# alibasaran/die-e

Hardware: AMD Instinct MI355X
Metric: self-play games/sec (higher is better)
Workload: dtype bf16

## Files before the change

die-e_amd/csrc/mcts_kernels.hip:

```cpp
#include <hip/hip_runtime.h>
#include <stdint.h>

#include <algorithm>
#include <type_traits>

#include "bg_device.h"
#include "nn_device.h"
#include "launch.h"
#include "mcts_device.h"
#include "search_iter_device.h"
#include "search_types.h"
#include "wave_ops.h"

namespace diee {

__device__ __forceinline__ void backprop(const Tree& T, size_t base, uint32_t idx, float v) {
    while (idx != kNone) {
        T.visits[base + idx] += 1.0f;
        T.value[base + idx] += v;
        idx = T.parent[base + idx];
    }
}

__device__ __forceinline__ void backprop_path(const Tree& T, size_t base, uint32_t my_node, int lane, uint32_t len, float v) {
// ... 419 lines not shown
            cn[SC_EXPANSIONS] += 1; cn[SC_CHILDREN] += (uint32_t)k;
            if ((uint32_t)k > cn[SC_MAX_CHILDREN]) cn[SC_MAX_CHILDREN] = (uint32_t)k;
        }
    }
    }
    EX_STAMP(4);
    meet();
    EX_STAMP(5);
    if constexpr (!TWO) bp_section();
    }
    };
    if constexpr (!TWO) commit();
    if constexpr (TWO == 2) {
        if (!main_wave) {
            commit();
            if (lane == 0) { sc_all.hand[0] = expanded ? 1u : 0u; sc_all.hand[1] = new_meta; sc_all.hand[2] = new_first; }
            __syncthreads();
            return;
        }
    }
    EX_STAMP(6);
    if (next_it != kNoNext) {
        meet();
        EX_STAMP(7);
        if constexpr (TWO) {
            select_slot(T, S, G, slot, seg, lane, next_it, c, P.quirks, cn, &rh, &l0, [&](uint32_t nd, uint32_t& nm, uint32_t& nf) {
                if (committed || nd != node) return false;
                commit();
                if (!expanded) return false;
                meet();
                nm = new_meta; nf = new_first;
                return true;
            });
        } else {
            select_slot(T, S, G, slot, seg, lane, next_it, c, P.quirks, cn, &rh, &l0);
        }
        EX_STAMP(8);
    }
    if constexpr (TWO) if (!committed) commit();
    if (lane == 0) store_counters(S, slot, cn);
#ifdef DIEE_EXPAND_STAMPS
    if (threadIdx.x == 0) atomicAdd(&g_expand_stamps[15], 1ull);
#endif
}

template <bool PRE, int TWO = 0>
__global__ __launch_bounds__(TWO ? 128 : 64) void k_expand(Tree T, Slots S, Segs G, uint32_t n, uint32_t it, SearchParams P,
                                                           uint32_t next_it, float c) {
    __shared__ ExpandScratchOf<PRE, TWO> sc_all;
    expand_body<PRE, TWO>(T, S, G, n, it, P, next_it, c, blockIdx.x, sc_all);
}

constexpr int kTailSpin = 1 << 20;
__device__ __forceinline__ bool tail_meet(uint32_t* word, uint32_t n, bool hit, int lane, uint32_t* err, uint32_t& misses, bool absent = false) {
    if (n == 1) { misses = hit ? 0u : 1u; return true; }
    __threadfence();
    uint32_t v = 0;
    if (lane == 0) {
        if (!absent) atomicAdd(word, hit ? 1u : 0x10001u);
        int spins = 0;
        for (;;) {
            v = __hip_atomic_load(word, __ATOMIC_RELAXED, __HIP_MEMORY_SCOPE_AGENT);
            if ((v & 0xffffu) >= n) break;
            if (++spins > kTailSpin) { atomicOr(err, 4u); v = 0xffffffffu; break; }
            __builtin_amdgcn_s_sleep(2);
        }
    }
    v = (uint32_t)__builtin_amdgcn_readfirstlane((int)v);
    __builtin_amdgcn_fence(__ATOMIC_ACQUIRE, "agent");
    misses = v >> 16;
    return v != 0xffffffffu;
}

#ifdef DIEE_TAIL_STAMPS
__device__ unsigned long long g_tail_stamps[8];
#define TL_STAMP(i) do { const unsigned long long tn_ = __builtin_readcyclecounter(); if (threadIdx.x == 0) atomicAdd(&g_tail_stamps[i], tn_ - tl_prev_); tl_prev_ = __builtin_readcyclecounter(); } while (0)
#define TL_COUNT(i) do { if (threadIdx.x == 0) atomicAdd(&g_tail_stamps[i], 1ull); } while (0)
extern "C" int diee_dev_tail_stamps(unsigned long long* out, int reset) {
    if (out && hipMemcpyFromSymbol(out, HIP_SYMBOL(g_tail_stamps), sizeof(unsigned long long) * 8) != hipSuccess) return 1;
    if (reset) { unsigned long long z[8] = {0}; if (hipMemcpyToSymbol(HIP_SYMBOL(g_tail_stamps), z, sizeof(z)) != hipSuccess) return 1; }
    return 0;
}
#else
#define TL_STAMP(i) do {} while (0)
#define TL_COUNT(i) do {} while (0)
#endif
struct TailArgs { Tail L; uint32_t q; };

struct TailTree {
    float vis[kTailLdsNodes], val[kTailLdsNodes], pri[kTailLdsNodes], cval[kTailLdsNodes];
    uint32_t meta[kTailLdsNodes], fc[kTailLdsNodes], crow[kTailLdsNodes];
};
struct TailLds {
    TailTree t;
    float vvis[kTailLdsNodes], vval[kTailLdsNodes];
    WaveScratch ws;
    float lgs[22 * 64];
    float raw[kMaxPlays];
    uint16_t code[kMaxPlays];
    uint32_t cand[64];
};
static_assert(sizeof(TailLds) <= 160 * 1024, "one workgroup per CU");

struct TreeLds : StagedStats {
    TailTree& t;
    struct Hdr { uint32_t meta, first_child; __device__ __forceinline__ uint32_t bits() const { return meta; } };
    __device__ __forceinline__ Hdr hdr(uint32_t i) const { return i < cap ? Hdr{t.meta[i], t.fc[i]} : Hdr{T.meta[base + i], T.first_child[base + i]}; }
    __device__ __forceinline__ static uint32_t nch(const Hdr& h) { return meta_nch(h.meta); }
    __device__ __forceinline__ static uint32_t fc(const Hdr& h) { return h.first_child; }
    __device__ __forceinline__ uint32_t leaf_meta(uint32_t, const Hdr& h) const { return h.meta; }
    __device__ __forceinline__ void set_header(uint32_t i, uint32_t m, uint32_t f) const {
        if (i < cap) { t.meta[i] = m; t.fc[i] = f; }
        T.meta[base + i] = m; T.first_child[base + i] = f;
    }
};

__global__ __launch_bounds__(64) void k_tail(Tree T, Slots S, Segs G, uint32_t n, SearchParams P, float c, TailArgs A) {
    extern __shared__ __attribute__((aligned(16))) char tail_smem[];
    uint32_t slot = blockIdx.x;
    if (gridDim.x == 8u * n) { if ((blockIdx.x & 7u) != 0u) return; slot = blockIdx.x >> 3; }
    if (slot >= n) return;
    const Tail& L = A.L;
    const int lane = threadIdx.x;
    if (L.state[1] != 0u) return;
#ifdef DIEE_TAIL_STAMPS
    unsigned long long tl_prev_ = __builtin_readcyclecounter();
#endif
    TL_COUNT(7);
    uint32_t it = L.state[0];
    TailLds& D = *reinterpret_cast<TailLds*>(tail_smem);
    const size_t base = (size_t)slot * T.node_cap;
    uint32_t* crow_g = L.crow + (size_t)slot * T.node_cap;
    float* cval_g = L.cval + (size_t)slot * T.node_cap;
    const TreeLds X{{T, base, kTailLdsNodes, D.t.vis, D.t.val, D.t.pri}, D.t};
    const bool quirks = P.quirks != 0;
    SlotRecord R;
    R.load(T, S, G, slot, lane);
    bool all_sel = false;
    if (quirks && slot == R.seg_first) {
        const uint32_t g = R.seg_first + (uint32_t)lane;
        all_sel = __ballot(g < R.seg_end && S.sel[g] == kNone) == 0ull && R.seg_end - R.seg_first <= 64u;
    }
    const uint32_t nl = R.used < kTailLdsNodes ? R.used : kTailLdsNodes;
    for (uint32_t i = lane; i < nl; i += 64) {
        D.t.vis[i] = T.visits[base + i]; D.t.val[i] = T.value[base + i]; D.t.pri[i] = T.prior[base + i];
        D.t.meta[i] = T.meta[base + i]; D.t.fc[i] = T.first_child[base + i];
        D.t.crow[i] = crow_g[i]; D.t.cval[i] = cval_g[i];
    }
    __syncthreads();
    uint32_t ahead_hi = R.used;
    if (A.q > 0) {
        if (L.child_rows > 0) {
            for (uint32_t i = R.used + (uint32_t)lane; i < R.used + (uint32_t)kMaxPlays && i < kTailLdsNodes; i += 64) { D.t.crow[i] = 0; D.t.cval[i] = 0.0f; }
            __syncthreads();
        }
        const uint32_t pq = A.q - 1, nr = L.n_rows[pq] < L.rows ? L.n_rows[pq] : L.rows;
        for (uint32_t r = lane; r < nr; r += 64) {
            const uint32_t rn = L.rows_node[pq * L.rows + r];
            if ((rn >> 24) == slot) {
                const uint32_t node = rn & 0xFFFFFFu;
                const float cv = row_value(L.hv + (size_t)(pq * L.rows + r) * 72, S.wv);
                cval_g[node] = cv; crow_g[node] = pq * L.rows + r + 1u;
                if (node < kTailLdsNodes) { D.t.cval[node] = cv; D.t.crow[node] = pq * L.rows + r + 1u; }
                if (node >= ahead_hi) ahead_hi = node + 1u;
            }
        }
        ahead_hi = (uint32_t)wave_allmax_i32((int)ahead_hi);
        __syncthreads();
    }
    TL_STAMP(0);
    R.lst = load_state(&S.eval_states[slot]);
    const IterScratch scratch{&D.ws, D.lgs, D.raw, D.code};
    bool hit = false;
    uint32_t misses = 0;
    for (;;) {
        const uint32_t cr = R.lterm ? 0u : (R.leaf < kTailLdsNodes ? D.t.crow[R.leaf] : crow_g[R.leaf]);
        hit = R.lterm || cr != 0u;
        const uint32_t ring = (R.lterm || cr == 0u) ? 0u : cr - 1u;
        NetRowLoaded pre;
        pre.vh = value_head_load(L.hv + (size_t)ring * 72, S.wv, lane);
        softmax_load(L.logits + (size_t)ring * 1352, lane, pre.lg);
        if (!tail_meet(L.bar + it + A.q, n, hit, lane, S.overflow, misses, L.test_skip != 0u && slot == n - 1u && it + A.q + 1u == L.test_skip)) {
            if (lane == 0) { atomicMax(&L.state[1], 2u); L.host[1] = 2u; __threadfence_system(); }
            return;
        }
        TL_STAMP(1);
        if (misses != 0u) break;
        uint2 ifl = make_uint2(1u, 0u);
        if (R.lterm || (quirks && slot == R.seg_first && !all_sel)) ifl = *(const uint2*)(S.iter_flags + 2 * ((size_t)R.seg * G.iter_cap + it));
        search_iteration(S, R, X, pre, scratch, ifl, it, slot, lane, quirks, [&](uint32_t cl, float prj, uint32_t cm) {
            if (cl < kTailLdsNodes) {
                D.t.vis[cl] = 0.0f; D.t.val[cl] = 0.0f; D.t.pri[cl] = prj; D.t.meta[cl] = cm; D.t.fc[cl] = 0;
                if (cl >= ahead_hi) { D.t.crow[cl] = 0; D.t.cval[cl] = 0.0f; }
            }
        });
        if (it + 1 < L.iterations) {
            uint32_t* nflag = S.iter_flags + 2 * ((size_t)R.seg * G.iter_cap + it + 1);
            uint32_t node = 0, depth = 0, mine = lane == 0 ? 0u : kNone;
            TreeLds::Hdr h = X.hdr(0);
            float nvis = X.vis(0);
            for (;;) {
                const uint32_t k = X.nch(h);
                if (k == 0) break;
                node = X.fc(h) + select_level(X, X.fc(h), k, sqrtf(nvis), c, lane);
                ++depth;
                if ((uint32_t)lane == depth) mine = node;
                h = X.hdr(node); nvis = X.vis(node);
            }
            if (end_selection(S, R, X, node, depth, mine, h, lane)) {
                if (lane == 0 && quirks && R.sel == kNone) atomicAdd(&nflag[1], 1u);
            } else {
                R.sel = node;
                if (lane == 0) nflag[0] = 1u;
            }
        }
        ++it;
        __syncthreads();
        TL_STAMP(2); TL_COUNT(6);
        if (it >= L.iterations) break;
    }
    R.store(T, S, slot, lane);
    const bool done = it >= L.iterations;
    uint32_t mine_rows = 0, ncand = 0;
    if (!done) {
        const uint32_t room = L.rows - (misses < L.rows ? misses : L.rows);
        const uint32_t want0 = room / n + (slot < room % n ? 1u : 0u), want = want0 < 63u ? want0 : 63u;
        const uint32_t nu = R.used < kTailLdsNodes ? R.used : kTailLdsNodes;
        const bool redistribute = L.extra_rows > 0 && L.rollout_steps > 0 && n > 1 && room > 0 && room / n < 8u;
        const bool second_round = redistribute || L.child_rows > 0;
        const uint32_t want_x = !redistribute ? want : want + L.extra_rows < 63u ? want + L.extra_rows : 63u;
        if (want_x > 0 && L.rollout_steps > 0) {
            for (uint32_t i = lane; i < nu; i += 64) { D.vvis[i] = D.t.vis[i]; D.vval[i] = D.t.val[i]; }
            __syncthreads();
            const uint32_t demanded = hit ? kNone : R.leaf;
            uint32_t fruitless = 0;
            for (uint32_t step = 0; step < L.rollout_steps && ncand < want_x && fruitless < 8; ++step) {
                const VirtualDescent d = virtual_descent<true>(X, D.vvis, D.vval, nu, c, lane);
                const uint32_t node = d.node, cr = node < kTailLdsNodes ? D.t.crow[node] : crow_g[node];
                float x = 0.0f;
                bool fresh = false;
                if (d.bits & kMetaTerminal) x = finished_value(d.bits, R.root_player);
                else if (cr != 0) x = node < kTailLdsNodes ? D.t.cval[node] : cval_g[node];
                else if (!(d.bits & kDrained) && node != demanded) fresh = __ballot((uint32_t)lane < ncand && D.cand[lane] == node) == 0ull;
                if (fresh) { if (lane == 0) D.cand[ncand] = node; ++ncand; fruitless = 0; } else ++fruitless;
                virtual_visit(d, D.vvis, D.vval, nu, x, lane);
                __syncthreads();
            }
        }
        uint32_t nchild = 0;
        if (L.child_rows > 0 && !hit && !(R.leaf_meta & kDrained)) {
            int k = bg_legal_plays_wave(R.lst, &D.ws, lane, S.overflow);
            if (k > kMaxPlays || R.used + (uint32_t)k > T.node_cap) k = 0;
            nchild = (uint32_t)k < L.child_rows ? (uint32_t)k : L.child_rows;
            __syncthreads();
        }
        const uint32_t share = ncand < want ? ncand : want, dem = hit ? 0u : 1u;
        mine_rows = dem + share;
        uint32_t start = 0;
        if (lane == 0 && mine_rows) start = atomicAdd(&L.n_rows[A.q], mine_rows);
        start = (uint32_t)__builtin_amdgcn_readfirstlane((int)start);
        if ((uint32_t)lane < mine_rows && start + (uint32_t)lane < L.rows) {
            const uint32_t node = (dem && lane == 0) ? R.leaf : D.cand[(uint32_t)lane - dem];
            const uint32_t r = A.q * L.rows + start + (uint32_t)lane;
            store_state(&L.rows_state[r], (dem && lane == 0) ? R.lst : load_state(&T.state[base + node]));
            L.rows_node[r] = (slot << 24) | node;
        }
        uint32_t extra = 0;
        if (second_round) {
            uint32_t unused_;
            const bool met = tail_meet(L.bar2 + A.q, n, true, lane, S.overflow, unused_);
            const uint32_t more = redistribute ? ncand - share : 0u;
            extra = met ? nchild + more : 0u;
            uint32_t start2 = 0;
            if (lane == 0 && extra) {
                start2 = atomicAdd(&L.n_rows[A.q], extra);
                const uint32_t fit = start2 >= L.rows ? 0u : extra < L.rows - start2 ? extra : L.rows - start2;
                if (fit < extra) atomicSub(&L.n_rows[A.q], extra - fit);
            }
            start2 = (uint32_t)__builtin_amdgcn_readfirstlane((int)start2);
            extra = start2 >= L.rows ? 0u : extra < L.rows - start2 ? extra : L.rows - start2;
            for (uint32_t j = (uint32_t)lane; j < extra; j += 64) {
                const uint32_t r = A.q * L.rows + start2 + j;
                if (j < nchild) {
                    BgState cs = R.lst;
                    int d0, d1;
                    draw_dice(R.seed, R.gid, R.rnd, it + 1u, j, d0, d1);
                    bg_apply_dev(cs, D.ws.play[j], d0, d1);
                    store_state(&L.rows_state[r], cs);
                    L.rows_node[r] = (slot << 24) | (R.used + j);
                } else {
                    const uint32_t node = D.cand[share + (j - nchild)];
                    store_state(&L.rows_state[r], load_state(&T.state[base + node]));
                    L.rows_node[r] = (slot << 24) | node;
                }
            }
        }
        R.cn[SC_NN_ROWS] += mine_rows + extra;
        if (lane == 0 && share + extra) atomicAdd(&L.state[3], share + extra);
    }
    if (lane == 0) store_counters(S, slot, R.cn);
    TL_STAMP(3);
    if (slot == 0 && lane == 0 && !done) L.n_dem[A.q] = misses;
    if (slot == 0 && lane == 0) {
        const uint32_t was = atomicMax(&L.state[1], done ? 1u : 0u);
        const uint32_t now = was > (done ? 1u : 0u) ? was : (done ? 1u : 0u);
        L.state[0] = it;
        if (!done) L.state[2] += 1u;
        L.host[0] = it; L.host[1] = now; L.host[2] = A.q;
        __threadfence_system();
    }
}

constexpr int kFreeSpinFew = 48, kFreeFewGames = 64;
constexpr uint32_t kFreeRowBits = 12;
struct FreeArgs { Free F; uint32_t q; };
#ifdef DIEE_TAIL_STAMPS
__device__ unsigned long long g_free_stamps[16];
#define FR_STAMP(i) do { const unsigned long long tn_ = __builtin_readcyclecounter(); if (threadIdx.x == 0) atomicAdd(&g_free_stamps[i], tn_ - fr_prev_); fr_prev_ = __builtin_readcyclecounter(); } while (0)
#define FR_COUNT(i, k) do { if (threadIdx.x == 0) atomicAdd(&g_free_stamps[i], (unsigned long long)(k)); } while (0)
extern "C" int diee_dev_free_stamps(unsigned long long* out, int reset) {
    if (out && hipMemcpyFromSymbol(out, HIP_SYMBOL(g_free_stamps), sizeof(unsigned long long) * 16) != hipSuccess) return 1;
    if (reset) { unsigned long long z[16] = {0}; if (hipMemcpyToSymbol(HIP_SYMBOL(g_free_stamps), z, sizeof(z)) != hipSuccess) return 1; }
    return 0;
}
#else
#define FR_STAMP(i) do {} while (0)
#define FR_COUNT(i, k) do {} while (0)
#endif
constexpr uint32_t kFreeLdsNodeBytes = 32;
__host__ __device__ __forceinline__ constexpr uint32_t free_hdr(uint32_t meta, uint32_t first_child) {
    return (meta & 0xE0000000u) | (((meta >> 16) & 0x1ffu) << 20) | (first_child & 0xFFFFFu);
}
__host__ __device__ __forceinline__ constexpr uint32_t hdr_nch(uint32_t h) { return (h >> 20) & 0x1ffu; }
__host__ __device__ __forceinline__ constexpr uint32_t hdr_fc(uint32_t h) { return h & 0xFFFFFu; }
__host__ __device__ constexpr size_t free_lds_bytes(uint32_t ln) {
    return (size_t)ln * kFreeLdsNodeBytes + sizeof(WaveScratch) + sizeof(float) * kMaxPlays + sizeof(uint16_t) * kMaxPlays + sizeof(uint32_t) * 64u;
}
struct TreeF : StagedStats {
    uint32_t* lhdr;
    struct Hdr { uint32_t w; __device__ __forceinline__ uint32_t bits() const { return w; } };
    __device__ __forceinline__ Hdr hdr(uint32_t i) const { return Hdr{i < cap ? lhdr[i] : free_hdr(T.meta[base + i], T.first_child[base + i])}; }
    __device__ __forceinline__ static uint32_t nch(const Hdr& h) { return hdr_nch(h.w); }
    __device__ __forceinline__ static uint32_t fc(const Hdr& h) { return hdr_fc(h.w); }
    __device__ __forceinline__ uint32_t leaf_meta(uint32_t i, const Hdr&) const { return T.meta[base + i]; }
    __device__ __forceinline__ void set_header(uint32_t i, uint32_t m, uint32_t f) const {
        if (i < cap) lhdr[i] = free_hdr(m, f);
        T.meta[base + i] = m; T.first_child[base + i] = f;
    }
};
__device__ __forceinline__ uint32_t free_load(const uint32_t* p) { return __hip_atomic_load(p, __ATOMIC_RELAXED, __HIP_MEMORY_SCOPE_AGENT); }

__global__ __launch_bounds__(64) void k_free(Tree T, Slots S, Segs G, uint32_t n, SearchParams P, float c, FreeArgs A) {
    extern __shared__ __attribute__((aligned(16))) char free_smem[];
    const uint32_t slot = blockIdx.x;
    if (slot >= n) return;
    const Free& F = A.F;
    const int lane = threadIdx.x;
    if (F.state[0] != 0u) return;
    uint32_t it = F.prog[slot];
    if (it >= F.iterations) { if (lane == 0) F.wish_n[slot] = it << 8; return; }
    const uint32_t active0 = A.q == 0 ? n : F.state[4];
    const uint32_t active = active0 ? active0 : 1u;
    const bool few = active * 8u <= n || active <= 8u;
    const uint32_t iter_cap = few ? 64u * F.iter_cap : F.iter_cap;
#ifdef DIEE_TAIL_STAMPS
    unsigned long long fr_prev_ = __builtin_readcyclecounter();
    const unsigned long long fr_t0_ = fr_prev_;
#endif
    FR_COUNT(8, 1);
    const uint32_t ln = F.lds_nodes;
    float* lvis = (float*)free_smem; float* lval = lvis + ln; float* lpri = lval + ln;
    float* vvis = lpri + ln; float* vval = vvis + ln;
    float* lcval = vval + ln;
    uint32_t* lhdr = (uint32_t*)(lcval + ln); uint32_t* lcrow = lhdr + ln;
    WaveScratch& ws = *reinterpret_cast<WaveScratch*>(lcrow + ln);
    float* raw = reinterpret_cast<float*>(&ws + 1);
    uint16_t* code = reinterpret_cast<uint16_t*>(raw + kMaxPlays);
    uint32_t* cand = reinterpret_cast<uint32_t*>(code + kMaxPlays);
    float* lgs = (float*)&ws.keyA[0];
    const size_t base = (size_t)slot * T.node_cap;
    uint32_t* crow_g = F.crow + base;
    float* cval_g = F.cval + base;
    const TreeF X{{T, base, ln, lvis, lval, lpri}, lhdr};
    const bool quirks = P.quirks != 0;
    SlotRecord R;
    R.load(T, S, G, slot, lane);
    uint32_t fsel = 0;
    if (quirks && slot == R.seg_first) {
        uint32_t m = 0;
        for (uint32_t g = R.seg_first + (uint32_t)lane; g < R.seg_end; g += 64) {
            const uint32_t f = F.first_sel[g];
            m = f == kNone ? 0x7fffffffu : (f > m ? f : m);
            if (f == kNone) break;
        }
        fsel = (uint32_t)wave_allmax_i32((int)m);
    }
    const uint32_t nl = R.used < ln ? R.used : ln;
    for (uint32_t i0 = 0; i0 < nl; i0 += 256) {
        float a[4], b[4], p[4], cv4[4]; uint32_t m[4], f[4], r[4];
#pragma unroll
        for (int u = 0; u < 4; ++u) {
            const uint32_t i = i0 + 64u * u + (uint32_t)lane;
            const size_t gi = base + (i < nl ? i : 0u);
// ... 25 lines not shown
    auto batch_progress = [&]() {
        int m = 0x7fffffff;
        for (uint32_t g = R.seg_first + (uint32_t)lane; g < R.seg_end; g += 64) { const int v = (int)free_load(&F.prog[g]); m = v < m ? v : m; }
        return (uint32_t)(-wave_allmax_i32(-m));
    };
    R.lst = load_state(&S.eval_states[slot]);
    const IterScratch scratch{&ws, lgs, raw, code};
    FR_STAMP(0);
    bool have = false, stalled = false;
    uint32_t minprog = 0;
    auto net_row = [&](uint32_t cr_) {
        NetRowLoaded p;
        const size_t ring = (size_t)(((cr_ - 1u) >> kFreeRowBits) % F.ring) * F.rows + ((cr_ - 1u) & ((1u << kFreeRowBits) - 1u));
        p.vh = value_head_load(F.hv + ring * 72, S.wv, lane);
        softmax_load(F.logits + ring * 1352, lane, p.lg);
        return p;
    };
    uint32_t cr = R.lterm ? 0u : crow_of(R.leaf);
    NetRowLoaded pre;
    if (!R.lterm && at_hand(cr)) pre = net_row(cr);
    uint32_t ran = 0;
    for (;; ++ran) {
        have = R.lterm || at_hand(cr);
        if (!have) break;
        if (ran >= iter_cap) { stalled = true; break; }
        uint32_t* iflag = S.iter_flags + 2 * ((size_t)R.seg * G.iter_cap + it);
        const bool need_cnt = quirks && slot == R.seg_first && it < fsel;
        const bool need_any = R.lterm && (quirks || slot == R.seg_first);
        uint2 ifl = make_uint2(1u, 0u);
        if (need_any || need_cnt) {
            bool fin = false;
            const int spins = n <= (uint32_t)kFreeFewGames ? kFreeSpinFew : 1;
            for (int spin = 0; spin < spins; ++spin) {
                if (!need_cnt && (iflag[0] != 0u || free_load(&iflag[0]) != 0u)) { ifl.x = 1u; fin = true; break; }
                if (minprog < it) minprog = batch_progress();
                if (minprog >= it) {
                    ifl.x = free_load(&iflag[0]); ifl.y = free_load(&iflag[1]);
                    fin = true;
                    break;
                }
                __builtin_amdgcn_s_sleep(8);
            }
            if (!fin) { stalled = true; break; }
        }
        FR_STAMP(1);
        search_iteration(S, R, X, pre, scratch, ifl, it, slot, lane, quirks, [&](uint32_t cl, float prj, uint32_t cm) {
            crow_g[cl] = 0u;
            if (cl < ln) { lvis[cl] = 0.0f; lval[cl] = 0.0f; lpri[cl] = prj; lhdr[cl] = free_hdr(cm, 0u); lcrow[cl] = 0; }
        });
        FR_STAMP(2);
        uint32_t published = 0;
        if (it + 1 < F.iterations) {
            uint32_t* nflag = S.iter_flags + 2 * ((size_t)R.seg * G.iter_cap + it + 1);
            uint32_t node = 0, depth = 0, mine = lane == 0 ? 0u : kNone;
            TreeF::Hdr h = X.hdr(0);
            float nvis = X.vis(0);
            for (;;) {
                const uint32_t k = X.nch(h), fcn = X.fc(h);
                if (k == 0) break;
                const float sq = sqrtf(nvis);
                if (k <= 64u && fcn + k <= ln) {
                    const bool valid = (uint32_t)lane < k;
                    const uint32_t ci = fcn + (valid ? (uint32_t)lane : 0u);
                    const float vis = lvis[ci];
                    const uint32_t ch = lhdr[ci];
                    const float sc_ = puct_score(vis, lval[ci], lpri[ci], sq, c);
                    const unsigned long long nans = __ballot(valid && sc_ != sc_);
                    const int lastnan = nans ? 63 - __clzll((long long)nans) : -1;
                    const bool comp = valid && sc_ == sc_ && lane > lastnan;
                    const float mx = wave_allmax_f32(comp ? sc_ : -INFINITY);
                    const unsigned long long win = __ballot(comp && sc_ == mx);
                    const int chosen = win ? 63 - __clzll((long long)win) : lastnan;
                    node = fcn + (uint32_t)chosen;
                    ++depth;
                    if ((uint32_t)lane == depth) mine = node;
                    h.w = (uint32_t)__builtin_amdgcn_readlane((int)ch, chosen);
                    nvis = __builtin_bit_cast(float, __builtin_amdgcn_readlane(__builtin_bit_cast(int, vis), chosen));
                    continue;
                }
                node = fcn + select_level(X, fcn, k, sq, c, lane);
                ++depth;
                if ((uint32_t)lane == depth) mine = node;
                h = X.hdr(node); nvis = X.vis(node);
            }
            if (end_selection(S, R, X, node, depth, mine, h, lane)) {
                if (lane == 0 && quirks && R.sel == kNone) published = atomicAdd(&nflag[1], 1u);
            } else {
                if (lane == 0) {
                    if (nflag[0] == 0u) published = atomicOr(&nflag[0], 1u);
                    if (R.sel == kNone) F.first_sel[slot] = it + 1u;
                }
                R.sel = node;
            }
            cr = R.lterm ? 0u : crow_of(R.leaf);
            if (!R.lterm && at_hand(cr)) pre = net_row(cr);
        }
        ++it;
        __syncthreads();
        if (lane == 0) {
            asm volatile("" :: "v"(published) : "memory");
            atomicExch(&F.prog[slot], it);
        }
        FR_STAMP(3); FR_COUNT(9, 1);
        if (it >= F.iterations) break;
    }
    R.store(T, S, slot, lane);
    const bool done = it >= F.iterations;
    uint32_t nw = 0;
    const bool dem = !done && !stalled && !have;
    if (!done) {
        uint32_t* wl = F.wish + (size_t)slot * kFreeWish;
        if (dem) { if (lane == 0) wl[0] = R.leaf; nw = 1; }
        uint32_t want0 = F.cand_max < kFreeWish - 1u ? F.cand_max : kFreeWish - 1u;
        uint32_t steps_max = F.rollout_steps;
        if (few && want0) {
            const uint32_t room = (F.rows > active ? F.rows - active : 0u) / active;
            want0 = room + 1u < kFreeWish - 1u ? (room + 1u > want0 ? room + 1u : want0) : kFreeWish - 1u;
            steps_max = 2u * F.rollout_steps + 8u;
        }
        const uint32_t want = few ? want0 : (want0 > ran / 2u + 1u ? want0 - ran / 2u : (want0 ? 1u : 0u));
        uint32_t ncand = 0;
        if (want > 0 && steps_max > 0) {
            const uint32_t nu = R.used < ln ? R.used : ln;
            for (uint32_t i0 = 0; i0 < nu; i0 += 256) {
                float a[4], b[4];
#pragma unroll
                for (int u = 0; u < 4; ++u) { const uint32_t i = i0 + 64u * u + (uint32_t)lane; a[u] = lvis[i < nu ? i : 0u]; b[u] = lval[i < nu ? i : 0u]; }
#pragma unroll
                for (int u = 0; u < 4; ++u) { const uint32_t i = i0 + 64u * u + (uint32_t)lane; if (i < nu) { vvis[i] = a[u]; vval[i] = b[u]; } }
            }
            __syncthreads();
            const uint32_t demanded = dem ? R.leaf : kNone;
            uint32_t fruitless = 0;
            const uint32_t h0 = X.hdr(0).w, k0 = hdr_nch(h0), fc0 = hdr_fc(h0);
            const bool resident = R.used <= ln && k0 >= 1u && k0 <= 64u;
            if (resident) {
                auto rl_u = [](uint32_t v_, int l_) { return (uint32_t)__builtin_amdgcn_readlane((int)v_, l_); };
                auto rl_f = [](float v_, int l_) { return __builtin_bit_cast(float, __builtin_amdgcn_readlane(__builtin_bit_cast(int, v_), l_)); };
                const bool rc = (uint32_t)lane < k0;
                const uint32_t rci = fc0 + (rc ? (uint32_t)lane : 0u);
                float r_vis = vvis[0], c_vis = vvis[rci], c_val = vval[rci];
                const float c_pri = lpri[rci], c_cval = lcval[rci];
                const uint32_t c_hdr = lhdr[rci], c_crow = lcrow[rci];
                uint32_t my_cand = kNone;
                for (uint32_t step = 0; step < steps_max && ncand < want && fruitless < 8; ++step) {
                    auto last_max = [&](bool comp, float sc_, uint32_t k_) {
                        const float mx = wave_allmax_f32(comp ? sc_ : -INFINITY);
                        const unsigned long long win = __ballot(comp && sc_ == mx);
                        return win ? 63 - __clzll((long long)win) : (int)k_ - 1;
                    };
                    int j0;
                    {
                        const float sq = __builtin_amdgcn_sqrtf(r_vis);
                        const float sc_ = puct_score_approx(c_vis, c_val, c_pri, sq, c);
                        j0 = last_max(rc && sc_ == sc_, sc_, k0);
                    }
                    uint32_t node = fc0 + (uint32_t)j0, depth = 1, mine = kNone, mt = h0;
                    uint32_t hn = rl_u(c_hdr, j0), ncr = rl_u(c_crow, j0);
                    float pvis = rl_f(c_vis, j0), pval = 0.0f, ncv = rl_f(c_cval, j0), mvis = 0.0f, mval = 0.0f;
                    for (;;) {
                        mt = hn;
                        const uint32_t k = hdr_nch(mt);
                        if (k == 0) break;
                        const uint32_t fcn = hdr_fc(mt);
                        const float sq = __builtin_amdgcn_sqrtf(pvis);
                        if (k <= 64u) {
                            const bool valid = (uint32_t)lane < k;
                            const uint32_t ci = fcn + (valid ? (uint32_t)lane : 0u);
                            const float vis = vvis[ci], val = vval[ci], pr = lpri[ci], cv = lcval[ci];
                            const uint32_t h = lhdr[ci], cr = lcrow[ci];
                            const float sc_ = puct_score_approx(vis, val, pr, sq, c);
                            const int lw = last_max(valid && sc_ == sc_, sc_, k);
                            node = fcn + (uint32_t)lw;
                            hn = rl_u(h, lw); ncr = rl_u(cr, lw); pvis = rl_f(vis, lw); pval = rl_f(val, lw); ncv = rl_f(cv, lw);
                            ++depth;
                            if ((uint32_t)lane == depth) { mine = node; mvis = pvis; mval = pval; }
                            if (depth >= 63) break;
                            continue;
                        }
                        Best b{0.0f, -1};
                        for (uint32_t j = lane; j < k; j += 64) {
                            const uint32_t ci = fcn + j;
                            const float sc_ = puct_score_approx(vvis[ci], vval[ci], lpri[ci], sq, c);
                            if (sc_ == sc_ && (b.j < 0 || !(b.s > sc_))) { b.s = sc_; b.j = (int)j; }
                        }
                        b = wave_best(b);
                        node = fcn + (uint32_t)(b.j >= 0 ? b.j : (int)k - 1);
                        hn = lhdr[node]; ncr = lcrow[node]; pvis = vvis[node]; pval = vval[node]; ncv = lcval[node];
                        ++depth;
                        if ((uint32_t)lane == depth) { mine = node; mvis = pvis; mval = pval; }
                        if (depth >= 63) break;
                    }
                    float x = 0.0f;
                    bool fresh = false;
                    if (mt & kMetaTerminal) x = finished_value(mt, R.root_player);
                    else if (at_hand(ncr)) x = ncv;
                    else if (!(mt & kDrained) && node != demanded) fresh = __ballot((uint32_t)lane < ncand && my_cand == node) == 0ull;
                    if (fresh) { if ((uint32_t)lane == ncand) my_cand = node; if (lane == 0) wl[nw + ncand] = node; ++ncand; fruitless = 0; } else ++fruitless;
                    r_vis += 1.0f;
                    if (lane == j0) { c_vis += 1.0f; c_val += x; }
                    if (lane >= 2 && (uint32_t)lane <= depth) { vvis[mine] = mvis + 1.0f; vval[mine] = mval + x; }
                    __builtin_amdgcn_wave_barrier();
                    FR_COUNT(11, 1);
                }
            } else
            for (uint32_t step = 0; step < steps_max && ncand < want && fruitless < 8; ++step) {
                const VirtualDescent d = virtual_descent<false>(X, vvis, vval, nu, c, lane);
                const uint32_t node = d.node, cr = crow_of(node);
                float x = 0.0f;
                bool fresh = false;
                if (d.bits & kMetaTerminal) x = finished_value(d.bits, R.root_player);
                else if (at_hand(cr)) x = node < ln ? lcval[node] : cval_g[node];
                else if (!(d.bits & kDrained) && node != demanded) fresh = __ballot((uint32_t)lane < ncand && cand[lane] == node) == 0ull;
                if (fresh) { if (lane == 0) { cand[ncand] = node; wl[nw + ncand] = node; } ++ncand; fruitless = 0; } else ++fruitless;
                virtual_visit(d, vvis, vval, nu, x, lane);
                __syncthreads();
                FR_COUNT(11, 1);
            }
        }
        nw += ncand;
    }
    if (lane == 0) {
        F.wish_n[slot] = nw | (it << 8) | (dem ? 0x80000000u : 0u);
        store_counters(S, slot, R.cn);
    }
    FR_STAMP(4);
#ifdef DIEE_TAIL_STAMPS
    if (threadIdx.x == 0) atomicMax(&g_free_stamps[10], __builtin_readcyclecounter() - fr_t0_);
#endif
}

__global__ __launch_bounds__(256) void k_free_first_sel(const uint32_t* __restrict__ sel, uint32_t* __restrict__ first_sel, uint32_t n) {
    const uint32_t g = blockIdx.x * 256u + threadIdx.x;
    if (g < n) first_sel[g] = sel[g] == kNone ? kNone : 0u;
}

__global__ __launch_bounds__(1024) void k_free_pack(Free F, uint32_t n, uint32_t node_cap, uint32_t q, const BgState* __restrict__ arena) {
    const uint32_t kBoost = F.lag_boost < kFreeBoostMax ? F.lag_boost : kFreeBoostMax, kLagStep = F.lag_step ? F.lag_step : 1u;
    __shared__ uint32_t hist[kFreeWish + kFreeBoostMax + 2];
    __shared__ uint32_t wsum[16];
    __shared__ uint32_t s_full, s_rem, s_dem, s_undone, s_maxprog;
    const int tid = threadIdx.x, lane = tid & 63, wave = tid >> 6;
    if (F.state[0] != 0u) return;
    if (tid < (int)(kFreeWish + kFreeBoostMax + 2)) hist[tid] = 0;
    if (tid == 0) { s_dem = 0; s_undone = 0; s_maxprog = 0; }
    __syncthreads();
    const uint32_t rot = (q * 131u) % n;
    const uint32_t g = (uint32_t)tid < n ? ((uint32_t)tid + rot) % n : 0u;
    const uint32_t w = (uint32_t)tid < n ? F.wish_n[g] : ((F.iterations) << 8);
    const uint32_t cnt = (w & 0xffu) < kFreeWish ? (w & 0xffu) : kFreeWish, dem = (w >> 31) < cnt ? (w >> 31) : cnt, spec = cnt - dem, prog = (w >> 8) & 0x7fffffu;
    const bool undone = prog < F.iterations;
    if ((uint32_t)tid < n && undone) { atomicMax(&s_maxprog, prog); atomicAdd(&s_undone, 1u); if (dem) atomicAdd(&s_dem, 1u); }
    __syncthreads();
    const uint32_t lag = undone ? s_maxprog - prog : 0u;
    const uint32_t shift = kBoost - (lag / kLagStep < kBoost ? lag / kLagStep : kBoost);
    if ((uint32_t)tid < n) for (uint32_t r = 1; r <= spec; ++r) atomicAdd(&hist[r + shift], 1u);
    __syncthreads();
// ... 446 lines not shown
```

die-e_amd/csrc/search_iter_device.h:

```cpp
#pragma once
#include <hip/hip_runtime.h>
#include <stdint.h>

#include "bg_device.h"
#include "mcts_device.h"
#include "nn_device.h"
#include "search_types.h"
#include "wave_ops.h"

namespace diee {

__device__ __forceinline__ float puct_score(float vis, float val, float pr, float sq, float c) {
    const float q = vis == 0.0f ? 0.0f : val / vis;
    const float t = sq / (vis + 1.0f);
    const float u = c * t;
    const float w = u * pr;
    return q + w;
}
__device__ __forceinline__ float puct_score_approx(float vis, float val, float pr, float sq, float c) {
    const float q = vis == 0.0f ? 0.0f : val * __builtin_amdgcn_rcpf(vis);
    return q + (c * (sq * __builtin_amdgcn_rcpf(vis + 1.0f))) * pr;
}

struct Best { float s; int j; };
// ... 149 lines not shown
#pragma unroll
        for (int q = 0; q < 22; ++q) sc.lgs[lane + 64 * q] = pre.lg[q];
        __syncthreads();
        for (int j = lane; j < k; j += 64) {
            const uint32_t cd = bg_encode_dev(r0, r1, sc.ws->play[j]);
            sc.raw[j] = softmax_prob(sc.lgs[cd], smM, smInv); sc.code[j] = (uint16_t)cd;
        }
        __syncthreads();
        float pr[4];
#pragma unroll
        for (int r = 0; r < 4; ++r) pr[r] = lane + 64 * r < k ? sc.raw[lane + 64 * r] : 0.0f;
        float sum = 0.0f;
#pragma unroll
        for (int r = 0; r < 4; ++r) {
            const int kr = k - 64 * r < 64 ? k - 64 * r : 64;
            for (int j = 0; j < kr; ++j) sum += __builtin_bit_cast(float, __builtin_amdgcn_readlane(__builtin_bit_cast(int, pr[r]), j));
        }
        const uint32_t first = R.used;
        if (first + (uint32_t)k > T.node_cap) {
            if (lane == 0) atomicOr(S.overflow, 2u);
        } else {
            const uint32_t e = it + 1u;
            for (int j = lane; j < k; j += 64) {
                const uint32_t cl = first + (uint32_t)j;
                const size_t ci = X.base + cl;
                BgState cs = R.lst;
                int d0, d1;
                draw_dice(R.seed, R.gid, R.rnd, e, (uint32_t)j, d0, d1);
                bg_apply_dev(cs, sc.ws->play[j], d0, d1);
                store_state(&T.state[ci], cs);
                const float prj = sc.raw[j] / sum;
                const uint32_t cm = (uint32_t)sc.code[j] | meta_terminal_bits(cs);
                T.visits[ci] = 0.0f; T.value[ci] = 0.0f; T.prior[ci] = prj;
                T.parent[ci] = R.leaf; T.first_child[ci] = 0; T.meta[ci] = cm;
                on_child(cl, prj, cm);
            }
            const uint32_t nmeta = kDrained | ((uint32_t)k << 16) | (m0 & kMetaKeep);
            if (lane == 0) X.set_header(R.leaf, nmeta, first);
            R.used = first + (uint32_t)k;
            R.cn[SC_EXPANSIONS] += 1; R.cn[SC_CHILDREN] += (uint32_t)k;
            if ((uint32_t)k > R.cn[SC_MAX_CHILDREN]) R.cn[SC_MAX_CHILDREN] = (uint32_t)k;
        }
        __syncthreads();
    }
    if (!R.lterm) backprop_selection(X, R.plen, R.pnode, R.leaf, v, lane);
    if (quirks && slot == R.seg_first && ifl.y != 0u && lane == 0) {
        float rvis = X.vis(0), rval = X.val(0);
        for (uint32_t i = 0; i < ifl.y; ++i) { rvis += 1.0f; rval += R.rv0; }
        X.set_stats(0, rvis, rval);
    }
    __syncthreads();
}

template <class TreeX>
__device__ __forceinline__ bool end_selection(const Slots& S, SlotRecord& R, const TreeX& X, uint32_t node, uint32_t depth, uint32_t mine,
                                              const typename TreeX::Hdr& h, int lane) {
    const uint32_t npl = depth < S.path_cap ? depth + 1u : 0u;
    R.cn[SC_SELECTIONS] += 1; R.cn[SC_DEPTH_SUM] += depth;
    if (h.bits() & kMetaTerminal) {
        backprop_selection(X, npl, mine, node, finished_value(h.bits(), R.root_player), lane);
        R.cn[SC_TERMINAL] += 1;
        R.lterm = true;
        return true;
    }
    R.lterm = false; R.leaf = node; R.plen = npl; R.pnode = mine;
    R.leaf_meta = X.leaf_meta(node, h);
    R.lst = load_state(&X.T.state[X.base + node]);
    return false;
}

struct VirtualDescent { uint32_t node, depth, mine, bits; };
template <bool EXACT, class TreeX>
__device__ __forceinline__ VirtualDescent virtual_descent(const TreeX& X, const float* vvis, const float* vval, uint32_t nu, float c, int lane) {
    VirtualDescent d{0u, 0u, lane == 0 ? 0u : kNone, 0u};
    for (;;) {
        const typename TreeX::Hdr h = X.hdr(d.node);
        d.bits = h.bits();
        const uint32_t k = X.nch(h);
        if (k == 0) break;
        const uint32_t fcn = X.fc(h);
        const float nv = d.node < nu ? vvis[d.node] : X.T.visits[X.base + d.node];
        const float sq = EXACT ? sqrtf(nv) : __builtin_amdgcn_sqrtf(nv);
        Best b{0.0f, -1};
        for (uint32_t j = lane; j < k; j += 64) {
            const uint32_t ci = fcn + j;
            const float vis = ci < nu ? vvis[ci] : X.T.visits[X.base + ci], val = ci < nu ? vval[ci] : X.T.value[X.base + ci];
            const float sc_ = EXACT ? puct_score(vis, val, X.pri(ci), sq, c) : puct_score_approx(vis, val, X.pri(ci), sq, c);
            if (sc_ == sc_ && (b.j < 0 || !(b.s > sc_))) { b.s = sc_; b.j = (int)j; }
        }
        b = wave_best(b);
        d.node = fcn + (uint32_t)(b.j >= 0 ? b.j : (int)k - 1);
        ++d.depth;
        if ((uint32_t)lane == d.depth) d.mine = d.node;
        if (d.depth >= 63) break;
    }
    return d;
}
__device__ __forceinline__ void virtual_visit(const VirtualDescent& d, float* vvis, float* vval, uint32_t nu, float x, int lane) {
    if ((uint32_t)lane <= d.depth && d.mine < nu) { vvis[d.mine] += 1.0f; vval[d.mine] += x; }
}

}
```

Before: 127.2.

## Relax tail barrier fences and share lane-parallel selection and virtual descents

Drops the full threadfence before the cross-block tail barrier and the acquire fence after it. Ordering now relies on a dependency on the returned value of the flag atomics, which become atomicOr/atomicAdd, and on relaxed agent-scope loads of the iteration flags. The lane-parallel PUCT descent and the register-resident virtual descent loop move out of k_free into shared templates, and k_tail now uses them instead of per-level select_level calls and its generic virtual_descent loop. This is meant to cut barrier latency and selection cost in the tail kernel. The weaker fencing risks memory-ordering bugs across workgroups.

After: 127.8 (median of 6 runs). No clear change (+0.5%).

```diff
diff --git a/die-e_amd/csrc/mcts_kernels.hip b/die-e_amd/csrc/mcts_kernels.hip
--- a/die-e_amd/csrc/mcts_kernels.hip
+++ b/die-e_amd/csrc/mcts_kernels.hip
@@ -495,11 +495,13 @@
 }
 
 constexpr int kTailSpin = 1 << 20;
-__device__ __forceinline__ bool tail_meet(uint32_t* word, uint32_t n, bool hit, int lane, uint32_t* err, uint32_t& misses, bool absent = false) {
+__device__ __forceinline__ uint32_t free_load(const uint32_t* p) { return __hip_atomic_load(p, __ATOMIC_RELAXED, __HIP_MEMORY_SCOPE_AGENT); }
+__device__ __forceinline__ bool tail_meet(uint32_t* word, uint32_t n, bool hit, int lane, uint32_t* err, uint32_t& misses, uint32_t performed,
+                                          bool absent = false) {
     if (n == 1) { misses = hit ? 0u : 1u; return true; }
-    __threadfence();
     uint32_t v = 0;
     if (lane == 0) {
+        asm volatile("" :: "v"(performed) : "memory");
         if (!absent) atomicAdd(word, hit ? 1u : 0x10001u);
         int spins = 0;
         for (;;) {
@@ -510,7 +512,7 @@
         }
     }
     v = (uint32_t)__builtin_amdgcn_readfirstlane((int)v);
-    __builtin_amdgcn_fence(__ATOMIC_ACQUIRE, "agent");
+    asm volatile("" ::: "memory");
     misses = v >> 16;
     return v != 0xffffffffu;
 }
@@ -549,6 +551,8 @@
     TailTree& t;
     struct Hdr { uint32_t meta, first_child; __device__ __forceinline__ uint32_t bits() const { return meta; } };
     __device__ __forceinline__ Hdr hdr(uint32_t i) const { return i < cap ? Hdr{t.meta[i], t.fc[i]} : Hdr{T.meta[base + i], T.first_child[base + i]}; }
+    __device__ __forceinline__ Hdr lds_hdr(uint32_t i) const { return Hdr{t.meta[i], t.fc[i]}; }
+    __device__ __forceinline__ static Hdr lane_hdr(const Hdr& h, int l) { return Hdr{lane_u32(h.meta, l), lane_u32(h.first_child, l)}; }
     __device__ __forceinline__ static uint32_t nch(const Hdr& h) { return meta_nch(h.meta); }
     __device__ __forceinline__ static uint32_t fc(const Hdr& h) { return h.first_child; }
     __device__ __forceinline__ uint32_t leaf_meta(uint32_t, const Hdr& h) const { return h.meta; }
@@ -616,6 +620,7 @@
     const IterScratch scratch{&D.ws, D.lgs, D.raw, D.code};
     bool hit = false;
     uint32_t misses = 0;
+    uint32_t performed = 0;
     for (;;) {
         const uint32_t cr = R.lterm ? 0u : (R.leaf < kTailLdsNodes ? D.t.crow[R.leaf] : crow_g[R.leaf]);
         hit = R.lterm || cr != 0u;
@@ -623,14 +628,17 @@
         NetRowLoaded pre;
         pre.vh = value_head_load(L.hv + (size_t)ring * 72, S.wv, lane);
         softmax_load(L.logits + (size_t)ring * 1352, lane, pre.lg);
-        if (!tail_meet(L.bar + it + A.q, n, hit, lane, S.overflow, misses, L.test_skip != 0u && slot == n - 1u && it + A.q + 1u == L.test_skip)) {
+        if (!tail_meet(L.bar + it + A.q, n, hit, lane, S.overflow, misses, performed, L.test_skip != 0u && slot == n - 1u && it + A.q + 1u == L.test_skip)) {
             if (lane == 0) { atomicMax(&L.state[1], 2u); L.host[1] = 2u; __threadfence_system(); }
             return;
         }
         TL_STAMP(1);
         if (misses != 0u) break;
         uint2 ifl = make_uint2(1u, 0u);
-        if (R.lterm || (quirks && slot == R.seg_first && !all_sel)) ifl = *(const uint2*)(S.iter_flags + 2 * ((size_t)R.seg * G.iter_cap + it));
+        if (R.lterm || (quirks && slot == R.seg_first && !all_sel)) {
+            const uint32_t* iflag = S.iter_flags + 2 * ((size_t)R.seg * G.iter_cap + it);
+            ifl.x = free_load(&iflag[0]); ifl.y = free_load(&iflag[1]);
+        }
         search_iteration(S, R, X, pre, scratch, ifl, it, slot, lane, quirks, [&](uint32_t cl, float prj, uint32_t cm) {
             if (cl < kTailLdsNodes) {
                 D.t.vis[cl] = 0.0f; D.t.val[cl] = 0.0f; D.t.pri[cl] = prj; D.t.meta[cl] = cm; D.t.fc[cl] = 0;
@@ -639,22 +647,14 @@
         });
         if (it + 1 < L.iterations) {
             uint32_t* nflag = S.iter_flags + 2 * ((size_t)R.seg * G.iter_cap + it + 1);
-            uint32_t node = 0, depth = 0, mine = lane == 0 ? 0u : kNone;
-            TreeLds::Hdr h = X.hdr(0);
-            float nvis = X.vis(0);
-            for (;;) {
-                const uint32_t k = X.nch(h);
-                if (k == 0) break;
-                node = X.fc(h) + select_level(X, X.fc(h), k, sqrtf(nvis), c, lane);
-                ++depth;
-                if ((uint32_t)lane == depth) mine = node;
-                h = X.hdr(node); nvis = X.vis(node);
-            }
+            uint32_t node, depth, mine;
+            TreeLds::Hdr h;
+            select_descent(X, c, lane, node, depth, mine, h);
             if (end_selection(S, R, X, node, depth, mine, h, lane)) {
-                if (lane == 0 && quirks && R.sel == kNone) atomicAdd(&nflag[1], 1u);
+                if (lane == 0 && quirks && R.sel == kNone) performed = atomicAdd(&nflag[1], 1u);
             } else {
                 R.sel = node;
-                if (lane == 0) nflag[0] = 1u;
+                if (lane == 0) performed = atomicOr(&nflag[0], 1u);
             }
         }
         ++it;
@@ -677,6 +677,12 @@
             __syncthreads();
             const uint32_t demanded = hit ? kNone : R.leaf;
             uint32_t fruitless = 0;
+            if (virtual_resident(X, R.used)) {
+                uint32_t steps;
+                ncand = virtual_descents_resident<true>(X, D.vvis, D.vval, D.t.cval, D.t.crow, L.rollout_steps, want_x, demanded, R.root_player, c, lane, steps,
+                                                        [](uint32_t cr_) { return cr_ != 0u; }, [&](uint32_t j, uint32_t node) { if (lane == 0) D.cand[j] = node; });
+                __syncthreads();
+            } else
             for (uint32_t step = 0; step < L.rollout_steps && ncand < want_x && fruitless < 8; ++step) {
                 const VirtualDescent d = virtual_descent<true>(X, D.vvis, D.vval, nu, c, lane);
                 const uint32_t node = d.node, cr = node < kTailLdsNodes ? D.t.crow[node] : crow_g[node];
@@ -711,7 +717,7 @@
         uint32_t extra = 0;
         if (second_round) {
             uint32_t unused_;
-            const bool met = tail_meet(L.bar2 + A.q, n, true, lane, S.overflow, unused_);
+            const bool met = tail_meet(L.bar2 + A.q, n, true, lane, S.overflow, unused_, start);
             const uint32_t more = redistribute ? ncand - share : 0u;
             extra = met ? nchild + more : 0u;
             uint32_t start2 = 0;
@@ -783,6 +789,8 @@
     uint32_t* lhdr;
     struct Hdr { uint32_t w; __device__ __forceinline__ uint32_t bits() const { return w; } };
     __device__ __forceinline__ Hdr hdr(uint32_t i) const { return Hdr{i < cap ? lhdr[i] : free_hdr(T.meta[base + i], T.first_child[base + i])}; }
+    __device__ __forceinline__ Hdr lds_hdr(uint32_t i) const { return Hdr{lhdr[i]}; }
+    __device__ __forceinline__ static Hdr lane_hdr(const Hdr& h, int l) { return Hdr{lane_u32(h.w, l)}; }
     __device__ __forceinline__ static uint32_t nch(const Hdr& h) { return hdr_nch(h.w); }
     __device__ __forceinline__ static uint32_t fc(const Hdr& h) { return hdr_fc(h.w); }
     __device__ __forceinline__ uint32_t leaf_meta(uint32_t i, const Hdr&) const { return T.meta[base + i]; }
@@ -791,7 +799,6 @@
         T.meta[base + i] = m; T.first_child[base + i] = f;
     }
 };
-__device__ __forceinline__ uint32_t free_load(const uint32_t* p) { return __hip_atomic_load(p, __ATOMIC_RELAXED, __HIP_MEMORY_SCOPE_AGENT); }
 
 __global__ __launch_bounds__(64) void k_free(Tree T, Slots S, Segs G, uint32_t n, SearchParams P, float c, FreeArgs A) {
     extern __shared__ __attribute__((aligned(16))) char free_smem[];
@@ -923,37 +930,9 @@
         uint32_t published = 0;
         if (it + 1 < F.iterations) {
             uint32_t* nflag = S.iter_flags + 2 * ((size_t)R.seg * G.iter_cap + it + 1);
-            uint32_t node = 0, depth = 0, mine = lane == 0 ? 0u : kNone;
-            TreeF::Hdr h = X.hdr(0);
-            float nvis = X.vis(0);
-            for (;;) {
-                const uint32_t k = X.nch(h), fcn = X.fc(h);
-                if (k == 0) break;
-                const float sq = sqrtf(nvis);
-                if (k <= 64u && fcn + k <= ln) {
-                    const bool valid = (uint32_t)lane < k;
-                    const uint32_t ci = fcn + (valid ? (uint32_t)lane : 0u);
-                    const float vis = lvis[ci];
-                    const uint32_t ch = lhdr[ci];
-                    const float sc_ = puct_score(vis, lval[ci], lpri[ci], sq, c);
-                    const unsigned long long nans = __ballot(valid && sc_ != sc_);
-                    const int lastnan = nans ? 63 - __clzll((long long)nans) : -1;
-                    const bool comp = valid && sc_ == sc_ && lane > lastnan;
-                    const float mx = wave_allmax_f32(comp ? sc_ : -INFINITY);
-                    const unsigned long long win = __ballot(comp && sc_ == mx);
-                    const int chosen = win ? 63 - __clzll((long long)win) : lastnan;
-                    node = fcn + (uint32_t)chosen;
-                    ++depth;
-                    if ((uint32_t)lane == depth) mine = node;
-                    h.w = (uint32_t)__builtin_amdgcn_readlane((int)ch, chosen);
-                    nvis = __builtin_bit_cast(float, __builtin_amdgcn_readlane(__builtin_bit_cast(int, vis), chosen));
-                    continue;
-                }
-                node = fcn + select_level(X, fcn, k, sq, c, lane);
-                ++depth;
-                if ((uint32_t)lane == depth) mine = node;
-                h = X.hdr(node); nvis = X.vis(node);
-            }
+            uint32_t node, depth, mine;
+            TreeF::Hdr h;
+            select_descent(X, c, lane, node, depth, mine, h);
             if (end_selection(S, R, X, node, depth, mine, h, lane)) {
                 if (lane == 0 && quirks && R.sel == kNone) published = atomicAdd(&nflag[1], 1u);
             } else {
@@ -1003,77 +982,11 @@
             __syncthreads();
             const uint32_t demanded = dem ? R.leaf : kNone;
             uint32_t fruitless = 0;
-            const uint32_t h0 = X.hdr(0).w, k0 = hdr_nch(h0), fc0 = hdr_fc(h0);
-            const bool resident = R.used <= ln && k0 >= 1u && k0 <= 64u;
-            if (resident) {
-                auto rl_u = [](uint32_t v_, int l_) { return (uint32_t)__builtin_amdgcn_readlane((int)v_, l_); };
-                auto rl_f = [](float v_, int l_) { return __builtin_bit_cast(float, __builtin_amdgcn_readlane(__builtin_bit_cast(int, v_), l_)); };
-                const bool rc = (uint32_t)lane < k0;
-                const uint32_t rci = fc0 + (rc ? (uint32_t)lane : 0u);
-                float r_vis = vvis[0], c_vis = vvis[rci], c_val = vval[rci];
-                const float c_pri = lpri[rci], c_cval = lcval[rci];
-                const uint32_t c_hdr = lhdr[rci], c_crow = lcrow[rci];
-                uint32_t my_cand = kNone;
-                for (uint32_t step = 0; step < steps_max && ncand < want && fruitless < 8; ++step) {
-                    auto last_max = [&](bool comp, float sc_, uint32_t k_) {
-                        const float mx = wave_allmax_f32(comp ? sc_ : -INFINITY);
-                        const unsigned long long win = __ballot(comp && sc_ == mx);
-                        return win ? 63 - __clzll((long long)win) : (int)k_ - 1;
-                    };
-                    int j0;
-                    {
-                        const float sq = __builtin_amdgcn_sqrtf(r_vis);
-                        const float sc_ = puct_score_approx(c_vis, c_val, c_pri, sq, c);
-                        j0 = last_max(rc && sc_ == sc_, sc_, k0);
-                    }
-                    uint32_t node = fc0 + (uint32_t)j0, depth = 1, mine = kNone, mt = h0;
-                    uint32_t hn = rl_u(c_hdr, j0), ncr = rl_u(c_crow, j0);
-                    float pvis = rl_f(c_vis, j0), pval = 0.0f, ncv = rl_f(c_cval, j0), mvis = 0.0f, mval = 0.0f;
-                    for (;;) {
-                        mt = hn;
-                        const uint32_t k = hdr_nch(mt);
-                        if (k == 0) break;
-                        const uint32_t fcn = hdr_fc(mt);
-                        const float sq = __builtin_amdgcn_sqrtf(pvis);
-                        if (k <= 64u) {
-                            const bool valid = (uint32_t)lane < k;
-                            const uint32_t ci = fcn + (valid ? (uint32_t)lane : 0u);
-                            const float vis = vvis[ci], val = vval[ci], pr = lpri[ci], cv = lcval[ci];
-                            const uint32_t h = lhdr[ci], cr = lcrow[ci];
-                            const float sc_ = puct_score_approx(vis, val, pr, sq, c);
-                            const int lw = last_max(valid && sc_ == sc_, sc_, k);
-                            node = fcn + (uint32_t)lw;
-                            hn = rl_u(h, lw); ncr = rl_u(cr, lw); pvis = rl_f(vis, lw); pval = rl_f(val, lw); ncv = rl_f(cv, lw);
-                            ++depth;
-                            if ((uint32_t)lane == depth) { mine = node; mvis = pvis; mval = pval; }
-                            if (depth >= 63) break;
-                            continue;
-                        }
-                        Best b{0.0f, -1};
-                        for (uint32_t j = lane; j < k; j += 64) {
-                            const uint32_t ci = fcn + j;
-                            const float sc_ = puct_score_approx(vvis[ci], vval[ci], lpri[ci], sq, c);
-                            if (sc_ == sc_ && (b.j < 0 || !(b.s > sc_))) { b.s = sc_; b.j = (int)j; }
-                        }
-                        b = wave_best(b);
-                        node = fcn + (uint32_t)(b.j >= 0 ? b.j : (int)k - 1);
-                        hn = lhdr[node]; ncr = lcrow[node]; pvis = vvis[node]; pval = vval[node]; ncv = lcval[node];
-                        ++depth;
-                        if ((uint32_t)lane == depth) { mine = node; mvis = pvis; mval = pval; }
-                        if (depth >= 63) break;
-                    }
-                    float x = 0.0f;
-                    bool fresh = false;
-                    if (mt & kMetaTerminal) x = finished_value(mt, R.root_player);
-                    else if (at_hand(ncr)) x = ncv;
-                    else if (!(mt & kDrained) && node != demanded) fresh = __ballot((uint32_t)lane < ncand && my_cand == node) == 0ull;
-                    if (fresh) { if ((uint32_t)lane == ncand) my_cand = node; if (lane == 0) wl[nw + ncand] = node; ++ncand; fruitless = 0; } else ++fruitless;
-                    r_vis += 1.0f;
-                    if (lane == j0) { c_vis += 1.0f; c_val += x; }
-                    if (lane >= 2 && (uint32_t)lane <= depth) { vvis[mine] = mvis + 1.0f; vval[mine] = mval + x; }
-                    __builtin_amdgcn_wave_barrier();
-                    FR_COUNT(11, 1);
-                }
+            if (virtual_resident(X, R.used)) {
+                uint32_t steps;
+                ncand = virtual_descents_resident<false>(X, vvis, vval, lcval, lcrow, steps_max, want, demanded, R.root_player, c, lane, steps, at_hand,
+                                                         [&](uint32_t j, uint32_t node) { if (lane == 0) wl[nw + j] = node; });
+                FR_COUNT(11, steps);
             } else
             for (uint32_t step = 0; step < steps_max && ncand < want && fruitless < 8; ++step) {
                 const VirtualDescent d = virtual_descent<false>(X, vvis, vval, nu, c, lane);
diff --git a/die-e_amd/csrc/search_iter_device.h b/die-e_amd/csrc/search_iter_device.h
--- a/die-e_amd/csrc/search_iter_device.h
+++ b/die-e_amd/csrc/search_iter_device.h
@@ -225,6 +225,45 @@
     __syncthreads();
 }
 
+__device__ __forceinline__ uint32_t lane_u32(uint32_t v, int l) { return (uint32_t)__builtin_amdgcn_readlane((int)v, l); }
+__device__ __forceinline__ float lane_f32(float v, int l) { return __builtin_bit_cast(float, __builtin_amdgcn_readlane(__builtin_bit_cast(int, v), l)); }
+
+template <class TreeX>
+__device__ __forceinline__ uint32_t select_level_lanes(const TreeX& X, uint32_t fcn, uint32_t k, float sq, float c, int lane,
+                                                       typename TreeX::Hdr& h, float& nvis) {
+    const bool valid = (uint32_t)lane < k;
+    const uint32_t ci = fcn + (valid ? (uint32_t)lane : 0u);
+    const float vis = X.lvis[ci];
+    const typename TreeX::Hdr ch = X.lds_hdr(ci);
+    const float sc_ = puct_score(vis, X.lval[ci], X.lpri[ci], sq, c);
+    const unsigned long long nans = __ballot(valid && sc_ != sc_);
+    const int lastnan = nans ? 63 - __clzll((long long)nans) : -1;
+    const bool comp = valid && sc_ == sc_ && lane > lastnan;
+    const float mx = wave_allmax_f32(comp ? sc_ : -INFINITY);
+    const unsigned long long win = __ballot(comp && sc_ == mx);
+    const int chosen = win ? 63 - __clzll((long long)win) : lastnan;
+    h = TreeX::lane_hdr(ch, chosen);
+    nvis = lane_f32(vis, chosen);
+    return fcn + (uint32_t)chosen;
+}
+
+template <class TreeX>
+__device__ __forceinline__ void select_descent(const TreeX& X, float c, int lane, uint32_t& node, uint32_t& depth, uint32_t& mine,
+                                               typename TreeX::Hdr& h) {
+    node = 0; depth = 0; mine = lane == 0 ? 0u : kNone;
+    h = X.hdr(0);
+    float nvis = X.vis(0);
+    for (;;) {
+        const uint32_t k = X.nch(h), fcn = X.fc(h);
+        if (k == 0) break;
+        const float sq = sqrtf(nvis);
+        if (k <= 64u && fcn + k <= X.cap) node = select_level_lanes(X, fcn, k, sq, c, lane, h, nvis);
+        else { node = fcn + select_level(X, fcn, k, sq, c, lane); h = X.hdr(node); nvis = X.vis(node); }
+        ++depth;
+        if ((uint32_t)lane == depth) mine = node;
+    }
+}
+
 template <class TreeX>
 __device__ __forceinline__ bool end_selection(const Slots& S, SlotRecord& R, const TreeX& X, uint32_t node, uint32_t depth, uint32_t mine,
                                               const typename TreeX::Hdr& h, int lane) {
@@ -273,4 +312,89 @@
     if ((uint32_t)lane <= d.depth && d.mine < nu) { vvis[d.mine] += 1.0f; vval[d.mine] += x; }
 }
 
-}
+template <class TreeX>
+__device__ __forceinline__ bool virtual_resident(const TreeX& X, uint32_t used) {
+    const uint32_t k0 = X.nch(X.hdr(0));
+    return used <= X.cap && k0 >= 1u && k0 <= 64u;
+}
+template <bool EXACT, class TreeX, class AtHand, class Found>
+__device__ __forceinline__ uint32_t virtual_descents_resident(const TreeX& X, float* vvis, float* vval, const float* lcval, const uint32_t* lcrow,
+                                                              uint32_t steps_max, uint32_t want, uint32_t demanded, int root_player, float c, int lane,
+                                                              uint32_t& steps, AtHand&& at_hand, Found&& found) {
+    using Hdr = typename TreeX::Hdr;
+    auto vsqrt = [](float v_) { return EXACT ? sqrtf(v_) : __builtin_amdgcn_sqrtf(v_); };
+    auto score = [](float vis, float val, float pr, float sq, float c_) { return EXACT ? puct_score(vis, val, pr, sq, c_) : puct_score_approx(vis, val, pr, sq, c_); };
+    auto last_max = [](bool comp, float sc_, uint32_t k_) {
+        const float mx = wave_allmax_f32(comp ? sc_ : -INFINITY);
+        const unsigned long long win = __ballot(comp && sc_ == mx);
+        return win ? 63 - __clzll((long long)win) : (int)k_ - 1;
+    };
+    const Hdr h0 = X.hdr(0);
+    const uint32_t k0 = X.nch(h0), fc0 = X.fc(h0);
+    const bool rc = (uint32_t)lane < k0;
+    const uint32_t rci = fc0 + (rc ? (uint32_t)lane : 0u);
+    float r_vis = vvis[0], c_vis = vvis[rci], c_val = vval[rci];
+    const float c_pri = X.lpri[rci], c_cval = lcval[rci];
+    const Hdr c_hdr = X.lds_hdr(rci);
+    const uint32_t c_crow = lcrow[rci];
+    uint32_t my_cand = kNone, ncand = 0, fruitless = 0;
+    for (steps = 0; steps < steps_max && ncand < want && fruitless < 8; ++steps) {
+        int j0;
+        {
+            const float sq = vsqrt(r_vis);
+            const float sc_ = score(c_vis, c_val, c_pri, sq, c);
+            j0 = last_max(rc && sc_ == sc_, sc_, k0);
+        }
+        uint32_t node = fc0 + (uint32_t)j0, depth = 1, mine = kNone;
+        Hdr mt = h0, hn = TreeX::lane_hdr(c_hdr, j0);
+        uint32_t ncr = lane_u32(c_crow, j0);
+        float pvis = lane_f32(c_vis, j0), pval = 0.0f, ncv = lane_f32(c_cval, j0), mvis = 0.0f, mval = 0.0f;
+        for (;;) {
+            mt = hn;
+            const uint32_t k = X.nch(mt);
+            if (k == 0) break;
+            const uint32_t fcn = X.fc(mt);
+            const float sq = vsqrt(pvis);
+            if (k <= 64u) {
+                const bool valid = (uint32_t)lane < k;
+                const uint32_t ci = fcn + (valid ? (uint32_t)lane : 0u);
+                const float vis = vvis[ci], val = vval[ci], pr = X.lpri[ci], cv = lcval[ci];
+                const Hdr h = X.lds_hdr(ci);
+                const uint32_t cr = lcrow[ci];
+                const float sc_ = score(vis, val, pr, sq, c);
+                const int lw = last_max(valid && sc_ == sc_, sc_, k);
+                node = fcn + (uint32_t)lw;
+                hn = TreeX::lane_hdr(h, lw); ncr = lane_u32(cr, lw); pvis = lane_f32(vis, lw); pval = lane_f32(val, lw); ncv = lane_f32(cv, lw);
+                ++depth;
+                if ((uint32_t)lane == depth) { mine = node; mvis = pvis; mval = pval; }
+                if (depth >= 63) break;
+                continue;
+            }
+            Best b{0.0f, -1};
+            for (uint32_t j = lane; j < k; j += 64) {
+                const uint32_t ci = fcn + j;
+                const float sc_ = score(vvis[ci], vval[ci], X.lpri[ci], sq, c);
+                if (sc_ == sc_ && (b.j < 0 || !(b.s > sc_))) { b.s = sc_; b.j = (int)j; }
+            }
+            b = wave_best(b);
+            node = fcn + (uint32_t)(b.j >= 0 ? b.j : (int)k - 1);
+            hn = X.lds_hdr(node); ncr = lcrow[node]; pvis = vvis[node]; pval = vval[node]; ncv = lcval[node];
+            ++depth;
+            if ((uint32_t)lane == depth) { mine = node; mvis = pvis; mval = pval; }
+            if (depth >= 63) break;
+        }
+        float x = 0.0f;
+        bool fresh = false;
+        if (mt.bits() & kMetaTerminal) x = finished_value(mt.bits(), root_player);
+        else if (at_hand(ncr)) x = ncv;
+        else if (!(mt.bits() & kDrained) && node != demanded) fresh = __ballot((uint32_t)lane < ncand && my_cand == node) == 0ull;
+        if (fresh) { if ((uint32_t)lane == ncand) my_cand = node; found(ncand, node); ++ncand; fruitless = 0; } else ++fruitless;
+        r_vis += 1.0f;
+        if (lane == j0) { c_vis += 1.0f; c_val += x; }
+        if (lane >= 2 && (uint32_t)lane <= depth) { vvis[mine] = mvis + 1.0f; vval[mine] = mval + x; }
+        __builtin_amdgcn_wave_barrier();
+    }
+    return ncand;
+}
+
+}
```
